# AkshayJha22/Cross-Sectional-Momentum-Strategy-Replication-Backtesting-Framework

Measured on AMD Instinct MI355X. Metric: asset-periods backtested/sec (1/2/4/8 GPU) + % HBM peak BW; decile match %, higher is better.
Workload: dtype f64

## Files before the change

### cross-sectional-momentum-strategy-replication-backtesting-framework_amd/csrc/signal.hip

```cpp
#include "csm_common.h"
#include "scan.h"
#include "shard.h"


#define PROBE_M 8
#define PROBE_DEN 8
__device__ __forceinline__ bool tail_probe(const double* __restrict__ P,
                                           const int64_t* __restrict__ month_start, int T_m,
                                           int64_t N, int64_t T_d) {
  static_assert(PROBE_M == 8, "the month spacing is a shift");
  const int lane = threadIdx.x & 63;
  const int64_t cs = N / 128;
  double x[PROBE_M][2];
  bool in[PROBE_M];
#pragma unroll
  for (int i = 0; i < PROBE_M; ++i) {
    const int m = (int)(((int64_t)(2 * i + 1) * T_m) >> 4);
    const int64_t d0 = month_start[m] < 0 ? 0 : month_start[m];
    const int64_t d1 = month_start[m + 1] < T_d ? month_start[m + 1] : T_d;
    in[i] = d1 > d0;
#pragma unroll
    for (int j = 0; j < 2; ++j)
      x[i][j] = in[i] ? P[(d1 - 1) * N + (2 * lane + j) * cs] : 0.0;
  }
  int gaps = 0, tot = 0;
#pragma unroll
  for (int i = 0; i < PROBE_M; ++i)
#pragma unroll
    for (int j = 0; j < 2; ++j) {
      gaps += __popcll(__ballot(in[i] && !(x[i][j] == x[i][j])));
      tot += in[i] ? 64 : 0;
    }
  return gaps * PROBE_DEN <= tot;
}

struct HaloArgs {
  int H, F, before, after;
  uint8_t* flags;
};
#define HALO_BATCH 8
template <int MAXD, int VEC, int NBUF, int BW, bool SH, bool BL, int JC = 0, bool HALO = false>
__global__ __launch_bounds__(64 * BW) void k_signal(
    const double* __restrict__ P, const int64_t* __restrict__ month_start, int T_m, int64_t N,
    int J, int skip, double* __restrict__ PMo, double* __restrict__ R, double* __restrict__ M,
    double* __restrict__ NR, const double* __restrict__ carry, const double* __restrict__ next_pm,
    double* __restrict__ carry_out, int64_t T_d, uint16_t* __restrict__ IDS, HaloArgs ha,
    int probe) {
  static_assert(!HALO || (SH && VEC == 2), "the halo prologue: shard passes, paired lanes");
  if (probe && tail_probe(P, month_start, T_m, N, T_d)) return;
  typedef typename RowT<VEC>::T VT;
  extern __shared__ __attribute__((aligned(16))) double ring_lds[];
  const int W = J + skip;
  const int tid = threadIdx.x;
  const int64_t a0 = ((int64_t)blockIdx.x * 64 * BW + tid) * VEC;
  const bool live = a0 < N;
  const int RS = 64 * VEC * BW;
  ScanLane sl[VEC];
  int* shc = reinterpret_cast<int*>(ring_lds + W * RS);
#pragma unroll
  for (int k = 0; k < VEC; ++k) {
    scan_init(sl[k], ring_lds + VEC * tid + k, RS, W, HALO ? nullptr : carry, N, a0 + k, live);
    if (SH) {
      shc[VEC * tid + k] = 0;
      shc[RS + VEC * tid + k] = -1;
      shc[2 * RS + VEC * tid + k] = -1;
    }
  }
  double npmh[VEC];
  if constexpr (HALO) {
    constexpr int HU = HALO_BATCH;
    const int64_t* ms = month_start;
    const int H = ha.H, F = ha.F, HF = H + F;
    const int64_t as = live ? a0 : 0;
    const int lane = tid & 63, wv = tid >> 6;
    const int64_t aw = a0 - 2 * lane;
    double* hpw = ring_lds + (size_t)W * RS + (size_t)(3 * RS) / 2;
    uint16_t* wl = reinterpret_cast<uint16_t*>(hpw + HU * RS) + wv * (HU * 128);
    int nh[VEC], fv[VEC], lv[VEC];
#pragma unroll
    for (int c = 0; c < VEC; ++c) { nh[c] = 0; fv[c] = -1; lv[c] = -1; npmh[c] = absent_val(); }
    for (int j0 = 0; j0 < HF; j0 += HU) {
      double2 xl[HU];
#pragma unroll
      for (int u = 0; u < HU; ++u) {
        const int j = j0 + u;
        const int m = j < H ? j : j + T_m;
        xl[u] = make_double2(absent_val(), absent_val());
        if (j < HF) {
          const int64_t d0 = ms[m], d1 = ms[m + 1];
          if (d1 > d0) xl[u] = *reinterpret_cast<const double2*>(P + (d1 - 1) * N + as);
        }
      }
      int nit = 0;
#pragma unroll
      for (int u = 0; u < HU; ++u) {
        *reinterpret_cast<double2*>(hpw + u * RS + 2 * tid) = xl[u];
#pragma unroll
        for (int c = 0; c < VEC; ++c) {
          const double x = comp(xl[u], c);
          const bool need = live && j0 + u < HF && !(x == x);
          const uint64_t mk = __ballot(need);
          if (need) wl[nit + lane_prefix(mk)] = (uint16_t)(u * 128 + 2 * lane + c);
          nit += __popcll(mk);
        }
      }
      __builtin_amdgcn_wave_barrier();
      for (int it0 = 0; it0 < nit; it0 += 128) {
        int item[2], u[2];
        int64_t d0[2], d1[2];
        double xs[2][HALO_WALK];
#pragma unroll
        for (int h = 0; h < 2; ++h) {
          const int it = it0 + 64 * h + lane;
          item[h] = it < nit ? (int)wl[it] : -1;
          u[h] = item[h] >> 7;
          const int j = j0 + (item[h] < 0 ? 0 : u[h]);
          const int m = j < H ? j : j + T_m;
          d0[h] = ms[m];
          d1[h] = ms[m + 1];
          const int64_t a = aw + (item[h] & 127);
#pragma unroll
          for (int k = 0; k < HALO_WALK; ++k) {
            const int64_t d = d1[h] - 2 - k;
            xs[h][k] = (item[h] >= 0 && d >= d0[h]) ? P[d * N + a] : absent_val();
          }
        }
#pragma unroll
        for (int h = 0; h < 2; ++h) {
          if (item[h] < 0) continue;
          const int64_t a = aw + (item[h] & 127);
          const double xlast = hpw[u[h] * RS + 128 * wv + (item[h] & 127)];
          bool p = !is_absent(xlast), got = false;
          double x = 0.0;
#pragma unroll
          for (int k = 0; k < HALO_WALK; ++k) {
            if (!got && xs[h][k] == xs[h][k]) { x = xs[h][k]; got = true; }
            p |= !is_absent(xs[h][k]);
          }
          if (!got && d1[h] - 1 - HALO_WALK > d0[h]) {
            const double y = halo_month_price(P, d0[h], d1[h] - 1 - HALO_WALK, N, a);
            if (y == y) { x = y; got = true; }
            p |= !is_absent(y);
          }
          hpw[u[h] * RS + 128 * wv + (item[h] & 127)] = got ? x : (p ? qnan() : absent_val());
        }
      }
      __syncthreads();
#pragma unroll
      for (int u = 0; u < HU; ++u) {
        const int j = j0 + u;
        if (j >= HF) break;
#pragma unroll
        for (int c = 0; c < VEC; ++c) {
          const double x = hpw[u * RS + 2 * tid + c];
          if (j < H) {
            if (live && !is_absent(x)) {
              if (!isnan_d(x)) { if (fv[c] < 0) fv[c] = nh[c]; lv[c] = nh[c]; }
              ++nh[c];
              scan_shadow(sl[c], x, j, ring_lds + VEC * tid + c, RS, W, J);
            }
          } else if (is_absent(npmh[c])) {
            npmh[c] = x;
          }
        }
      }
      __syncthreads();
    }
#pragma unroll
    for (int c = 0; c < VEC; ++c) {
      sl[c].prev = -1;
      uint8_t fl = 0;
      if (ha.before && !(fv[c] >= 0 && lv[c] - fv[c] >= W)) fl |= 1;
      if (ha.after && is_absent(npmh[c])) fl |= 2;
      if (live && ha.flags) ha.flags[a0 + c] = fl;
    }
    month_start += H;
  }
  const double* base = P + (live ? a0 : 0);
  const int64_t rstride = N;
  static_assert(!BL || VEC == 2, "buffer loads: paired lanes");
  const int voff = (int)((live ? a0 : 0) * 8);
  auto load_month = [&](VT (&buf)[MAXD], int mm) {
    mm = mm < T_m ? mm : T_m - 1;
    const int64_t f0 = month_start[mm], nn = month_start[mm + 1] - f0;
    if constexpr (BL) {
      typedef unsigned int u32x4 __attribute__((ext_vector_type(4)));
      const __amdgpu_buffer_rsrc_t rs = __builtin_amdgcn_make_buffer_rsrc(
          (void*)(P + f0 * N), (short)0, (int)(nn * N * 8), 0x00020000);
#pragma unroll
      for (int k = 0; k < MAXD; ++k) {
        const u32x4 w = __builtin_amdgcn_raw_buffer_load_b128(rs, voff + k * (int)(N * 8), 0, 0);
        buf[k] = *reinterpret_cast<const VT*>(&w);
      }
    } else {
      const int64_t pad = nn > 0 ? nn - 1 : (f0 > 0 ? -1 : 0);
#pragma unroll
      for (int k = 0; k < MAXD; ++k)
        buf[k] = *reinterpret_cast<const VT*>(base + (f0 + (k < nn ? k : pad)) * rstride);
    }
  };
  auto process = [&](const VT (&X)[MAXD], int m) {
    double pm[VEC];
    const int nnm = (int)(month_start[m + 1] - month_start[m]);
#pragma unroll
    for (int c = 0; c < VEC; ++c) {
      double last = 0.0;
      bool p = false, v = false;
#pragma unroll
      for (int k = 0; k < MAXD; ++k) {
        const double x = comp(X[k], c);
        const bool in = BL ? k < nnm : nnm > 0;
        const bool ok = in && x == x;
        p |= in && !is_absent(x);
        v |= ok;
        last = ok ? x : last;
      }
      pm[c] = p ? (v ? last : qnan()) : absent_val();
      if (SH && p) {
        int* q = shc + VEC * tid + c;
        q[0] += 1;
        if (q[RS] < 0) q[RS] = m;
        q[2 * RS] = m;
      }
    }
    if (live) {
      if (PMo && (!SH || shard_pm_kept(m, T_m, W))) {
        if (VEC == 2) *reinterpret_cast<double2*>(PMo + (int64_t)m * N + a0) = make_double2(pm[0], pm[VEC - 1]);
        else PMo[(int64_t)m * N + a0] = pm[0];
      }
      double mom[VEC];
      if constexpr (VEC == 2) {
        scan_step_pair<JC>(reinterpret_cast<ScanLane (&)[2]>(sl), reinterpret_cast<const double (&)[2]>(pm),
                       m, ring_lds + VEC * tid, RS, W, J, N, a0, R, M, NR,
                       reinterpret_cast<double (&)[2]>(mom));
      } else {
#pragma unroll
        for (int c = 0; c < VEC; ++c)
          mom[c] = scan_step(sl[c], pm[c], m, ring_lds + VEC * tid + c, RS, W, J, N, a0 + c, R, M, NR);
      }
      if (IDS) {
        if (VEC == 2)
          *reinterpret_cast<uint32_t*>(IDS + (int64_t)m * N + a0) =
              csm_fid(mom[0]) | (csm_fid(mom[VEC - 1]) << 16);
        else
          IDS[(int64_t)m * N + a0] = (uint16_t)csm_fid(mom[0]);
      }
    }
  };
  static_assert(NBUF == 2 || NBUF == 4, "two or four month buffers");
  VT A[MAXD], B[MAXD];
  if (NBUF == 2) {
    load_month(A, 0);
    for (int m = 0; m < T_m; m += 2) {
      load_month(B, m + 1);
      process(A, m);
      load_month(A, m + 2);
      if (m + 1 < T_m) process(B, m + 1);
    }
  } else {
    VT C[MAXD], D[MAXD];
    load_month(A, 0);
    load_month(B, 1);
    load_month(C, 2);
    for (int m = 0; m < T_m; m += 4) {
      load_month(D, m + 3);
      process(A, m);
      load_month(A, m + 4);
      if (m + 1 < T_m) process(B, m + 1);
      load_month(B, m + 5);
      if (m + 2 < T_m) process(C, m + 2);
      load_month(C, m + 6);
      if (m + 3 < T_m) process(D, m + 3);
    }
  }
  if (live) {
#pragma unroll
    for (int k = 0; k < VEC; ++k) {
      if constexpr (HALO) {
        if (sl[k].prev >= 0)
          NR[(int64_t)sl[k].prev * N + a0 + k] = pending_finish(npmh[k], sl[k].psff);
      } else {
        scan_finish(sl[k], ring_lds + VEC * tid + k, RS, W, N, a0 + k, NR, next_pm,
                    SH ? nullptr : carry_out);
      }
      if (SH) {
        const int* q = shc + VEC * tid + k;
        carry_out[a0 + k] = (double)q[0];
        carry_out[N + a0 + k] = (double)sl[k].prev;
        carry_out[2 * N + a0 + k] = sl[k].psff;
        carry_out[3 * N + a0 + k] = (double)q[RS];
        carry_out[4 * N + a0 + k] = (double)q[2 * RS];
      }
    }
  }
}

#define TAIL_U 8
#define TAIL_BACK 3

template <int MAXD, int BW, int JC>
__global__ __launch_bounds__(64 * BW) void k_signal_tail(
    const double* __restrict__ P, const int64_t* __restrict__ month_start, int T_m, int64_t N,
    int J, int skip, double* __restrict__ PMo, double* __restrict__ R, double* __restrict__ M,
    double* __restrict__ NR, const double* __restrict__ carry, const double* __restrict__ next_pm,
    double* __restrict__ carry_out, int64_t T_d, uint16_t* __restrict__ IDS,
    int probe) {
  if (probe && !tail_probe(P, month_start, T_m, N, T_d)) return;
  extern __shared__ __attribute__((aligned(16))) double ring_lds[];
  constexpr int U = TAIL_U, RS = 64 * BW, WA = 64;
  const int W = J + skip;
  const int tid = threadIdx.x, lane = tid & 63, wv = tid >> 6;
  const int64_t a0 = (int64_t)blockIdx.x * RS + tid;
  const bool live = a0 < N;
  const int64_t as = live ? a0 : 0;
  const int64_t aw = a0 - lane;
  const int64_t* ms = month_start;
  double* hp = ring_lds + (size_t)W * RS;
  double* hpw = hp + WA * wv;
  uint16_t* wl = reinterpret_cast<uint16_t*>(hp + U * RS) + wv * (2 * U * WA);
  uint16_t* wl2 = wl + U * WA;
  ScanLane sl;
  scan_init(sl, ring_lds + tid, RS, W, carry, N, a0, live);
  if (aw >= N) return;

  auto month_rows = [&](int m, int64_t& d0, int64_t& d1) {
    d0 = ms[m];
    d1 = ms[m + 1];
    d0 = d0 < 0 ? 0 : d0;
    d1 = d1 < T_d ? d1 : T_d;
  };
  auto load_last = [&](double (&xl)[U], int m0) {
#pragma unroll
    for (int u = 0; u < U; ++u) {
      xl[u] = absent_val();
      if (m0 + u < T_m) {
        int64_t d0, d1;
        month_rows(m0 + u, d0, d1);
        if (d1 > d0) xl[u] = P[(d1 - 1) * N + as];
      }
    }
  };
  auto fold = [&](double y, double& x, bool& got, bool& p) {
    if (!got && y == y) { x = y; got = true; }
    p |= !is_absent(y);
  };
  constexpr int K = MAXD - 1;
  struct Walk {
    int item, u, col;
    int64_t d0, d1;
    bool act;
  };
  auto issue = [&](auto& xs, Walk& w, const uint16_t* list, int it, int n, int m0) {
    constexpr int KK = sizeof(xs) / sizeof(double);
    w.act = it < n;
    w.item = w.act ? (int)list[it] : 0;
    w.u = w.item / WA;
    w.col = w.item % WA;
    month_rows(m0 + w.u, w.d0, w.d1);
    const int64_t a = aw + w.col;
#pragma unroll
    for (int k = 0; k < KK; ++k) {
      const int64_t d = w.d1 - 2 - k;
      xs[k] = (w.act && d >= w.d0) ? P[d * N + a] : absent_val();
    }
  };
  auto finish_back = [&](const double (&xs)[TAIL_BACK], const Walk& w, int& nb) {
    bool p = true, got = false;
    double x = 0.0;
#pragma unroll
    for (int k = 0; k < TAIL_BACK; ++k) fold(xs[k], x, got, p);
    const bool more = w.act && !got && w.d1 - 2 - TAIL_BACK >= w.d0;
    if (w.act && !more) hpw[w.u * RS + w.col] = got ? x : qnan();
    const uint64_t mk = __ballot(more);
    if (more) wl2[nb + lane_prefix(mk)] = (uint16_t)w.item;
    nb += __popcll(mk);
  };
  auto finish_month = [&](const double (&xs)[K], const Walk& w) {
    bool p = !is_absent(hpw[w.u * RS + w.col]), got = false;
    double x = 0.0;
#pragma unroll
    for (int k = 0; k < K; ++k) fold(xs[k], x, got, p);
    if (w.act) hpw[w.u * RS + w.col] = got ? x : (p ? qnan() : absent_val());
  };
  auto walk_months = [&](int i0, int n, int m0) {
    double XS[K], XT[K];
    Walk wb, wc;
    const bool two = i0 + 64 < n;
    issue(XS, wb, wl2, i0 + lane, n, m0);
    if (two) issue(XT, wc, wl2, i0 + 64 + lane, n, m0);
    finish_month(XS, wb);
    if (two) finish_month(XT, wc);
  };

  double xa[U], xb[U];
  load_last(xa, 0);
  for (int m0 = 0; m0 < T_m; m0 += U) {
    load_last(xb, m0 + U);
    int na = 0, nb = 0;
#pragma unroll
    for (int u = 0; u < U; ++u) {
      hp[u * RS + tid] = xa[u];
      bool in = false;
      if (m0 + u < T_m) {
        int64_t d0, d1;
        month_rows(m0 + u, d0, d1);
        in = d1 > d0;
      }
      const double x = xa[u];
      const bool need = live && in && !(x == x);
      const bool nb_ = need && is_absent(x), na_ = need && !nb_;
      const uint64_t mka = __ballot(na_), mkb = __ballot(nb_);
      const int item = u * WA + lane;
      if (na_) wl[na + lane_prefix(mka)] = (uint16_t)item;
      if (nb_) wl2[nb + lane_prefix(mkb)] = (uint16_t)item;
      na += __popcll(mka);
      nb += __popcll(mkb);
    }
    __builtin_amdgcn_wave_barrier();
    if (na + nb > 0) {
      double xs[TAIL_BACK];
      Walk wa;
      int db = nb < 128 ? nb : 128;
      issue(xs, wa, wl, lane, na, m0);
      walk_months(0, db, m0);
      finish_back(xs, wa, nb);
      for (int it0 = 64; it0 < na; it0 += 64) {
        issue(xs, wa, wl, it0 + lane, na, m0);
        finish_back(xs, wa, nb);
      }
      __builtin_amdgcn_wave_barrier();
      for (; db < nb; db += 128) walk_months(db, nb, m0);
    }
    __builtin_amdgcn_wave_barrier();
#pragma unroll 1
    for (int u = 0; u < U; ++u) {
      const int m = m0 + u;
      if (m >= T_m) break;
      if (!live) continue;
      const double pm = hp[u * RS + tid];
      if (PMo) PMo[(int64_t)m * N + a0] = pm;
      const double mom = scan_step<JC>(sl, pm, m, ring_lds + tid, RS, W, J, N, a0, R, M, NR);
      if (IDS) IDS[(int64_t)m * N + a0] = (uint16_t)csm_fid(mom);
    }
    __builtin_amdgcn_wave_barrier();
#pragma unroll
    for (int u = 0; u < U; ++u) xa[u] = xb[u];
  }
  if (live) scan_finish(sl, ring_lds + tid, RS, W, N, a0, NR, next_pm, carry_out);
}

static int g_tune_signal_vec = 2;
static int g_tune_signal_bwf = 0;
static int g_tune_signal_tail = 2;
static int g_tune_signal_j12 = 1;
#define SIGNAL_BWF_MIN_N (180 * 512)
static const TuneKnob g_knobs[] = {
    {"signal_vec", &g_tune_signal_vec, [](int v) { return v == 1 || v == 2; }},
    {"signal_bwf", &g_tune_signal_bwf, [](int v) { return v == 0 || v == 1 || v == 4; }},
    {"signal_j12", &g_tune_signal_j12, [](int v) { return v == 0 || v == 1; }},
    {"signal_tail", &g_tune_signal_tail, [](int v) { return v >= 0 && v <= 2; }},
};
int csm_tune_signal(const char* key, int value) { return tune_set(g_knobs, key, value); }

int signal_launch(csm_ctx* ctx, const char* who, const double* P, int64_t T_d, int64_t N,
                  const int64_t* month_start, int32_t T_m, int32_t max_month_days, int32_t J,
                  int32_t skip, double* PM, double* R, double* M, double* NR, const double* carry,
                  const double* next_pm, double* carry_out, bool sh, uint16_t* ids,
                  const HaloArgs* halo) {
  int r = prep(ctx);
  if (r) return r;
  if (sh && (!PM || !carry_out || T_m < 1))
    return set_err(ctx, CSM_E_INVAL, "%s: a shard pass needs PM and state, and at least one month",
                   who);
  if (!P || !month_start || !M || !NR || N <= 0 || T_d < 0 || T_m < 0 || J < 1 || skip < 0 ||
      J + skip > 256 || max_month_days < 1)
    return set_err(ctx, CSM_E_INVAL, "%s: bad arguments (N=%lld T_m=%d J=%d skip=%d)", who,
                   (long long)N, T_m, J, skip);
  if (max_month_days > 32)
    return set_err(ctx, CSM_E_INVAL, "%s: months longer than 32 days are not supported "
                   "(use csm_month_end + csm_momentum)", who);
  if (T_m == 0) return CSM_OK;
  if (T_d == 0)
    return set_err(ctx, CSM_E_INVAL, "%s: %d months and no day row", who, T_m);
  const int W = J + skip;
  const bool can2 = (N % 2 == 0) && aligned16(P) && (!PM || aligned16(PM)) && aligned16(M) &&
                    aligned16(NR) && (!R || aligned16(R));
  const int vec = (g_tune_signal_vec == 1 || !can2) ? 1 : 2;
  const size_t tlds = (size_t)(W + TAIL_U) * 128 * sizeof(double) + (size_t)2 * TAIL_U * 128 * sizeof(uint16_t);
  int tail = (!sh && !halo && can2 && tlds <= 160 * 1024) ? g_tune_signal_tail : 0;
  if (tail == 2 && N < (int64_t)SIGNAL_BWF_MIN_N) tail = 1;
  int probe_ = tail == 2;
  if (tail != 0) {
    const bool d23 = max_month_days <= 23, j12 = J == 12;
    const void* fn =
        d23 ? (j12 ? (const void*)k_signal_tail<23, 2, 12> : (const void*)k_signal_tail<23, 2, 0>)
            : (j12 ? (const void*)k_signal_tail<32, 2, 12> : (const void*)k_signal_tail<32, 2, 0>);
    if (tlds > 65536)
      HIP_CHECK(ctx, hipFuncSetAttribute(fn, hipFuncAttributeMaxDynamicSharedMemorySize, (int)tlds));
    const unsigned blocks = (unsigned)((N + 127) / 128);
    int T_m_ = T_m, J_ = J, skip_ = skip;
    int64_t N_ = N, T_d_ = T_d;
    void* args[] = {(void*)&P, (void*)&month_start, &T_m_, &N_, &J_, &skip_, (void*)&PM, (void*)&R,
                    (void*)&M, (void*)&NR, (void*)&carry, (void*)&next_pm, (void*)&carry_out, &T_d_,
                    (void*)&ids, &probe_};
    HIP_CHECK(ctx, hipLaunchKernel(fn, dim3(blocks), dim3(128), args, tlds, ctx->stream));
    LAUNCH_CHECK(ctx, who);
    if (tail == 1) return CSM_OK;
  }
  const bool fits4 = vec == 2 && max_month_days <= 23 && N * 8 * 32 < ((int64_t)1 << 31);
  const bool wide4 = fits4 && (g_tune_signal_bwf == 4 ||
                               (g_tune_signal_bwf == 0 && N >= (int64_t)SIGNAL_BWF_MIN_N));
  const int bw = wide4 ? 4 : 1;
  const size_t lds = (size_t)W * 64 * vec * bw * sizeof(double) +
                     (sh ? (size_t)3 * 64 * vec * bw * sizeof(int) : 0) +
                     (halo ? (size_t)HALO_BATCH * 64 * vec * bw * sizeof(double) +
                             (size_t)bw * HALO_BATCH * 128 * sizeof(uint16_t) : 0);
  const unsigned blocks = (unsigned)((N / vec + 64 * bw - 1) / (64 * bw));
  const void* fn = nullptr;
#define SIG1(V, SH_)                                                                            \
  (max_month_days <= 23 && V == 2 ? (const void*)k_signal<23, V, 4, 1, SH_, false>              \
   : max_month_days <= 24         ? (const void*)k_signal<24, V, 4, 1, SH_, false>              \
                                  : (const void*)k_signal<32, V, 4, 1, SH_, false>)
  const bool j12 = sh && J == 12 && g_tune_signal_j12;
  if (halo && !(sh && wide4))
    return set_err(ctx, CSM_E_INVAL, "%s: the fused halo prologue runs in the wide shard kernel "
                   "(even N >= %d, months of <= 23 days); use csm_shard_halo + "
                   "csm_signal_shard_halo", who, SIGNAL_BWF_MIN_N);
  if (halo)
    fn = j12 ? (const void*)k_signal<23, 2, 2, 4, true, true, 12, true>
             : (const void*)k_signal<23, 2, 2, 4, true, true, 0, true>;
  else if (wide4 && j12)
    fn = (const void*)k_signal<23, 2, 2, 4, true, true, 12>;
  else if (wide4)
    fn = sh ? (const void*)k_signal<23, 2, 2, 4, true, true> : (const void*)k_signal<23, 2, 2, 4, false, true>;
  else if (vec == 2)
    fn = sh ? SIG1(2, true) : SIG1(2, false);
  else
    fn = sh ? SIG1(1, true) : SIG1(1, false);
#undef SIG1
  if (lds > 65536)
    HIP_CHECK(ctx, hipFuncSetAttribute(fn, hipFuncAttributeMaxDynamicSharedMemorySize, (int)lds));
  {
    int T_m_ = T_m, J_ = J, skip_ = skip;
    int64_t N_ = N, T_d_ = T_d;
    HaloArgs ha = halo ? *halo : HaloArgs{0, 0, 0, 0, nullptr};
    void* args[] = {(void*)&P, (void*)&month_start, &T_m_, &N_, &J_, &skip_, (void*)&PM, (void*)&R,
                    (void*)&M, (void*)&NR, (void*)&carry, (void*)&next_pm, (void*)&carry_out, &T_d_,
                    (void*)&ids, (void*)&ha, &probe_};
    HIP_CHECK(ctx, hipLaunchKernel(fn, dim3(blocks), dim3(64 * bw), args, lds, ctx->stream));
  }
  LAUNCH_CHECK(ctx, who);
  return CSM_OK;
}

extern "C" {

int csm_signal(csm_ctx* ctx, const double* P, int64_t T_d, int64_t N, const int64_t* month_start,
               int32_t T_m, int32_t max_month_days, int32_t J, int32_t skip, double* PM, double* R,
               double* M, double* NR, const double* carry, const double* next_pm,
               double* carry_out) {
  return signal_launch(ctx, "csm_signal", P, T_d, N, month_start, T_m, max_month_days, J,
                       skip, PM, R, M, NR, carry, next_pm, carry_out);
}

int csm_signal_ids(csm_ctx* ctx, const double* P, int64_t T_d, int64_t N,
                   const int64_t* month_start, int32_t T_m, int32_t max_month_days,
                   int32_t min_month_days, int32_t J, int32_t skip, double* PM, double* R,
                   double* M, double* NR, uint16_t* ids) {
  if (!ids || (N % 4) != 0 || ((uintptr_t)ids & 7u) != 0)
    return set_err(ctx, CSM_E_INVAL, "csm_signal_ids: ids must be non-NULL and 8-B aligned, N %% 4 == 0 "
                   "(N=%lld)", (long long)N);
  (void)min_month_days;
  return signal_launch(ctx, "csm_signal_ids", P, T_d, N, month_start, T_m, max_month_days, J,
                       skip, PM, R, M, NR, nullptr, nullptr, nullptr, false, ids);
}

int csm_signal_shard(csm_ctx* ctx, const double* P, int64_t T_d, int64_t N,
                     const int64_t* month_start, int32_t T_m, int32_t max_month_days, int32_t J,
                     int32_t skip, double* PM, double* R, double* M, double* NR, double* state) {
  return signal_launch(ctx, "csm_signal_shard", P, T_d, N, month_start, T_m,
                       max_month_days, J, skip, PM, R, M, NR, nullptr, nullptr, state, true);
}

int csm_signal_shard_ids(csm_ctx* ctx, const double* P, int64_t T_d, int64_t N,
                         const int64_t* month_start, int32_t T_m, int32_t max_month_days,
                         int32_t J, int32_t skip, double* PM, double* R, double* M, double* NR,
                         double* state, uint16_t* ids) {
  if (!ids || (N % 4) != 0 || ((uintptr_t)ids & 7u) != 0)
    return set_err(ctx, CSM_E_INVAL, "csm_signal_shard_ids: needs ids, N %% 4 == 0, 8-B aligned ids");
  return signal_launch(ctx, "csm_signal_shard_ids", P, T_d, N, month_start, T_m,
                       max_month_days, J, skip, PM, R, M, NR, nullptr, nullptr, state, true, ids);
}

int csm_signal_halo(csm_ctx* ctx, const double* P, int64_t T_d, int64_t N,
                    const int64_t* month_start, int32_t H, int32_t T_m, int32_t F, int32_t before,
                    int32_t after, int32_t max_month_days, int32_t J, int32_t skip, double* PM,
                    double* R, double* M, double* NR, double* state, uint16_t* ids,
                    uint8_t* flags) {
  if (!flags || H < 0 || F < 0 || F > 8 || J + skip > 64)
    return set_err(ctx, CSM_E_INVAL, "csm_signal_halo: bad arguments (flags [N], H >= 0, "
                   "0 <= F <= 8, J + skip <= 64)");
  if (ids && ((N % 4) != 0 || ((uintptr_t)ids & 7u) != 0))
    return set_err(ctx, CSM_E_INVAL, "csm_signal_halo: ids need N %% 4 == 0, 8-B alignment");
  const HaloArgs ha{H, F, before ? 1 : 0, after ? 1 : 0, flags};
  return signal_launch(ctx, "csm_signal_halo", P, T_d, N, month_start, T_m, max_month_days, J,
                       skip, PM, R, M, NR, nullptr, nullptr, state, true, ids, &ha);
}

int csm_signal_shard_halo(csm_ctx* ctx, const double* P, int64_t T_d, int64_t N,
                          const int64_t* month_start, int32_t T_m, int32_t max_month_days,
                          int32_t J, int32_t skip, const double* carry, const double* next_pm,
                          double* PM, double* R, double* M, double* NR, double* state,
                          uint16_t* ids) {
  if (!carry || !next_pm)
    return set_err(ctx, CSM_E_INVAL, "csm_signal_shard_halo: needs the halo's carry and next_pm");
  if (ids && ((N % 4) != 0 || ((uintptr_t)ids & 7u) != 0))
    return set_err(ctx, CSM_E_INVAL, "csm_signal_shard_halo: ids need N %% 4 == 0, 8-B alignment");
  return signal_launch(ctx, "csm_signal_shard_halo", P, T_d, N, month_start, T_m, max_month_days,
                       J, skip, PM, R, M, NR, carry, next_pm, state, true, ids);
}

}
```

Measured before the change: 823.2 billion.

## Split signal tail kernel into producer loader waves and consumer scanner waves

The tail kernel now uses separate wave roles. Loader waves gather each month's last-valid prices into a double-buffered LDS staging area. Scanner waves then run the momentum scan on the previous batch, with block-level barriers handing each batch from loaders to scanners, so the gather latency overlaps the scan work. Day indices are narrowed to 32-bit, and a waves-per-EU occupancy hint is added. This costs twice the staging LDS, more threads per block and a __syncthreads per batch, and adds a guard that T_d fits in 32 bits.

```diff
diff --git a/cross-sectional-momentum-strategy-replication-backtesting-framework_amd/csrc/signal.hip b/cross-sectional-momentum-strategy-replication-backtesting-framework_amd/csrc/signal.hip
--- a/cross-sectional-momentum-strategy-replication-backtesting-framework_amd/csrc/signal.hip
+++ b/cross-sectional-momentum-strategy-replication-backtesting-framework_amd/csrc/signal.hip
@@ -297,46 +297,87 @@
 
 #define TAIL_U 8
 #define TAIL_BACK 3
-
-template <int MAXD, int BW, int JC>
-__global__ __launch_bounds__(64 * BW) void k_signal_tail(
+constexpr int TAIL_NS = 2;
+constexpr int TAIL_NL = 2;
+constexpr int TAIL_CPL = 1;
+constexpr int tail_waves_per_simd(int nw) { return nw == 4 ? 4 : 3; }
+
+template <int MAXD, int NS, int NL, int CPL, int JC>
+__global__ __launch_bounds__(64 * (NS + NL))
+__attribute__((amdgpu_waves_per_eu(tail_waves_per_simd(NS + NL)))) void k_signal_tail(
     const double* __restrict__ P, const int64_t* __restrict__ month_start, int T_m, int64_t N,
     int J, int skip, double* __restrict__ PMo, double* __restrict__ R, double* __restrict__ M,
     double* __restrict__ NR, const double* __restrict__ carry, const double* __restrict__ next_pm,
     double* __restrict__ carry_out, int64_t T_d, uint16_t* __restrict__ IDS,
     int probe) {
+  static_assert(NS % NL == 0 && (CPL == 1 || CPL == 2), "whole 64-column groups per loader wave");
   if (probe && !tail_probe(P, month_start, T_m, N, T_d)) return;
   extern __shared__ __attribute__((aligned(16))) double ring_lds[];
-  constexpr int U = TAIL_U, RS = 64 * BW, WA = 64;
+  constexpr int U = TAIL_U, RS = 64 * NS, CW = RS / NL, CP = CW / 64;
+  static_assert(U * CW <= 65536, "list items are 16-bit");
   const int W = J + skip;
-  const int tid = threadIdx.x, lane = tid & 63, wv = tid >> 6;
-  const int64_t a0 = (int64_t)blockIdx.x * RS + tid;
-  const bool live = a0 < N;
-  const int64_t as = live ? a0 : 0;
-  const int64_t aw = a0 - lane;
+  const int tid = threadIdx.x, lane = tid & 63;
+  const int wv = __builtin_amdgcn_readfirstlane(tid >> 6);
+  const bool scanner = wv < NS;
+  const int nbat = (T_m + U - 1) / U;
   const int64_t* ms = month_start;
   double* hp = ring_lds + (size_t)W * RS;
-  double* hpw = hp + WA * wv;
-  uint16_t* wl = reinterpret_cast<uint16_t*>(hp + U * RS) + wv * (2 * U * WA);
-  uint16_t* wl2 = wl + U * WA;
-  ScanLane sl;
-  scan_init(sl, ring_lds + tid, RS, W, carry, N, a0, live);
-  if (aw >= N) return;
-
-  auto month_rows = [&](int m, int64_t& d0, int64_t& d1) {
-    d0 = ms[m];
-    d1 = ms[m + 1];
-    d0 = d0 < 0 ? 0 : d0;
-    d1 = d1 < T_d ? d1 : T_d;
-  };
-  auto load_last = [&](double (&xl)[U], int m0) {
+  if (scanner) {
+    const int64_t a0 = (int64_t)blockIdx.x * RS + tid;
+    const bool live = a0 < N;
+    ScanLane sl;
+    scan_init(sl, ring_lds + tid, RS, W, carry, N, a0, live);
+    for (int k = 0; k <= nbat; ++k) {
+      if (k > 0 && live) {
+        const int m0 = (k - 1) * U;
+        const double* hb = hp + ((k - 1) & 1) * (U * RS) + tid;
+#pragma unroll 1
+        for (int u = 0; u < U; ++u) {
+          const int m = m0 + u;
+          if (m >= T_m) break;
+          const double pm = hb[u * RS];
+          if (PMo) PMo[(int64_t)m * N + a0] = pm;
+          const double mom = scan_step<JC>(sl, pm, m, ring_lds + tid, RS, W, J, N, a0, R, M, NR);
+          if (IDS) IDS[(int64_t)m * N + a0] = (uint16_t)csm_fid(mom);
+        }
+      }
+      if (k < nbat) __syncthreads();
+    }
+    if (live) scan_finish(sl, ring_lds + tid, RS, W, N, a0, NR, next_pm, carry_out);
+    return;
+  }
+  const int lw = wv - NS;
+  const int64_t aw = (int64_t)blockIdx.x * RS + (int64_t)lw * CW;
+  const bool wlive = aw < N;
+  bool lv[CP];
+  int64_t as[CP];
+#pragma unroll
+  for (int c = 0; c < CP; ++c) {
+    const int64_t a = aw + 64 * c + lane;
+    lv[c] = wlive && a < N;
+    as[c] = lv[c] ? a : 0;
+  }
+  double* hpw = hp + CW * lw;
+  uint16_t* wl = reinterpret_cast<uint16_t*>(hp + 2 * U * RS) + lw * (2 * U * CW);
+  uint16_t* wl2 = wl + U * CW;
+
+  auto month_rows = [&](int m, int& d0, int& d1) {
+    const int64_t e0 = ms[m], e1 = ms[m + 1];
+    d0 = (int)(e0 < 0 ? 0 : (e0 < T_d ? e0 : T_d));
+    d1 = (int)(e1 < T_d ? (e1 < 0 ? 0 : e1) : T_d);
+  };
+  auto load_last = [&](double (&xl)[U][CP], int m0) {
 #pragma unroll
     for (int u = 0; u < U; ++u) {
-      xl[u] = absent_val();
+#pragma unroll
+      for (int c = 0; c < CP; ++c) xl[u][c] = absent_val();
       if (m0 + u < T_m) {
-        int64_t d0, d1;
+        int d0, d1;
         month_rows(m0 + u, d0, d1);
-        if (d1 > d0) xl[u] = P[(d1 - 1) * N + as];
+        if (d1 > d0) {
+#pragma unroll
+          for (int c = 0; c < CP; ++c) xl[u][c] = P[(int64_t)(d1 - 1) * N + as[c]];
+        }
       }
     }
   };
@@ -347,21 +388,21 @@
   constexpr int K = MAXD - 1;
   struct Walk {
     int item, u, col;
-    int64_t d0, d1;
+    int d0, d1;
     bool act;
   };
   auto issue = [&](auto& xs, Walk& w, const uint16_t* list, int it, int n, int m0) {
     constexpr int KK = sizeof(xs) / sizeof(double);
     w.act = it < n;
     w.item = w.act ? (int)list[it] : 0;
-    w.u = w.item / WA;
-    w.col = w.item % WA;
+    w.u = w.item / CW;
+    w.col = w.item % CW;
     month_rows(m0 + w.u, w.d0, w.d1);
     const int64_t a = aw + w.col;
 #pragma unroll
     for (int k = 0; k < KK; ++k) {
-      const int64_t d = w.d1 - 2 - k;
-      xs[k] = (w.act && d >= w.d0) ? P[d * N + a] : absent_val();
+      const int d = w.d1 - 2 - k;
+      xs[k] = (w.act && d >= w.d0) ? P[(int64_t)d * N + a] : absent_val();
     }
   };
   auto finish_back = [&](const double (&xs)[TAIL_BACK], const Walk& w, int& nb) {
@@ -383,70 +424,70 @@
     if (w.act) hpw[w.u * RS + w.col] = got ? x : (p ? qnan() : absent_val());
   };
   auto walk_months = [&](int i0, int n, int m0) {
-    double XS[K], XT[K];
-    Walk wb, wc;
-    const bool two = i0 + 64 < n;
+    double XS[K];
+    Walk wb;
     issue(XS, wb, wl2, i0 + lane, n, m0);
-    if (two) issue(XT, wc, wl2, i0 + 64 + lane, n, m0);
-    finish_month(XS, wb);
-    if (two) finish_month(XT, wc);
-  };
-
-  double xa[U], xb[U];
-  load_last(xa, 0);
-  for (int m0 = 0; m0 < T_m; m0 += U) {
-    load_last(xb, m0 + U);
-    int na = 0, nb = 0;
-#pragma unroll
-    for (int u = 0; u < U; ++u) {
-      hp[u * RS + tid] = xa[u];
-      bool in = false;
-      if (m0 + u < T_m) {
-        int64_t d0, d1;
-        month_rows(m0 + u, d0, d1);
-        in = d1 > d0;
-      }
-      const double x = xa[u];
-      const bool need = live && in && !(x == x);
-      const bool nb_ = need && is_absent(x), na_ = need && !nb_;
-      const uint64_t mka = __ballot(na_), mkb = __ballot(nb_);
-      const int item = u * WA + lane;
-      if (na_) wl[na + lane_prefix(mka)] = (uint16_t)item;
-      if (nb_) wl2[nb + lane_prefix(mkb)] = (uint16_t)item;
-      na += __popcll(mka);
-      nb += __popcll(mkb);
-    }
-    __builtin_amdgcn_wave_barrier();
-    if (na + nb > 0) {
-      double xs[TAIL_BACK];
-      Walk wa;
-      int db = nb < 128 ? nb : 128;
-      issue(xs, wa, wl, lane, na, m0);
-      walk_months(0, db, m0);
-      finish_back(xs, wa, nb);
-      for (int it0 = 64; it0 < na; it0 += 64) {
-        issue(xs, wa, wl, it0 + lane, na, m0);
+    if constexpr (CPL == 2) {
+      double XT[K];
+      Walk wc;
+      const bool two = i0 + 64 < n;
+      if (two) issue(XT, wc, wl2, i0 + 64 + lane, n, m0);
+      finish_month(XS, wb);
+      if (two) finish_month(XT, wc);
+    } else {
+      finish_month(XS, wb);
+    }
+  };
+
+  double xa[U][CP];
+  if (wlive) load_last(xa, 0);
+  for (int k = 0; k < nbat; ++k) {
+    if (wlive) {
+      const int m0 = k * U;
+      hpw = hp + (k & 1) * (U * RS) + CW * lw;
+      int na = 0, nb = 0;
+#pragma unroll
+      for (int u = 0; u < U; ++u) {
+        bool in = false;
+        if (m0 + u < T_m) {
+          int d0, d1;
+          month_rows(m0 + u, d0, d1);
+          in = d1 > d0;
+        }
+#pragma unroll
+        for (int c = 0; c < CP; ++c) {
+          const double x = xa[u][c];
+          hpw[u * RS + 64 * c + lane] = x;
+          const bool need = lv[c] && in && !(x == x);
+          const bool nb_ = need && is_absent(x), na_ = need && !nb_;
+          const uint64_t mka = __ballot(na_), mkb = __ballot(nb_);
+          const int item = u * CW + 64 * c + lane;
+          if (na_) wl[na + lane_prefix(mka)] = (uint16_t)item;
+          if (nb_) wl2[nb + lane_prefix(mkb)] = (uint16_t)item;
+          na += __popcll(mka);
+          nb += __popcll(mkb);
+        }
+      }
+      load_last(xa, m0 + U);
+      __builtin_amdgcn_wave_barrier();
+      if (na + nb > 0) {
+        double xs[TAIL_BACK];
+        Walk wa;
+        constexpr int TRIP = 64 * CPL;
+        int db = nb < TRIP ? nb : TRIP;
+        issue(xs, wa, wl, lane, na, m0);
+        walk_months(0, db, m0);
         finish_back(xs, wa, nb);
-      }
-      __builtin_amdgcn_wave_barrier();
-      for (; db < nb; db += 128) walk_months(db, nb, m0);
-    }
-    __builtin_amdgcn_wave_barrier();
-#pragma unroll 1
-    for (int u = 0; u < U; ++u) {
-      const int m = m0 + u;
-      if (m >= T_m) break;
-      if (!live) continue;
-      const double pm = hp[u * RS + tid];
-      if (PMo) PMo[(int64_t)m * N + a0] = pm;
-      const double mom = scan_step<JC>(sl, pm, m, ring_lds + tid, RS, W, J, N, a0, R, M, NR);
-      if (IDS) IDS[(int64_t)m * N + a0] = (uint16_t)csm_fid(mom);
-    }
-    __builtin_amdgcn_wave_barrier();
-#pragma unroll
-    for (int u = 0; u < U; ++u) xa[u] = xb[u];
-  }
-  if (live) scan_finish(sl, ring_lds + tid, RS, W, N, a0, NR, next_pm, carry_out);
+        for (int it0 = 64; it0 < na; it0 += 64) {
+          issue(xs, wa, wl, it0 + lane, na, m0);
+          finish_back(xs, wa, nb);
+        }
+        __builtin_amdgcn_wave_barrier();
+        for (; db < nb; db += TRIP) walk_months(db, nb, m0);
+      }
+    }
+    __syncthreads();
+  }
 }
 
 static int g_tune_signal_vec = 2;
@@ -486,24 +527,28 @@
   const bool can2 = (N % 2 == 0) && aligned16(P) && (!PM || aligned16(PM)) && aligned16(M) &&
                     aligned16(NR) && (!R || aligned16(R));
   const int vec = (g_tune_signal_vec == 1 || !can2) ? 1 : 2;
-  const size_t tlds = (size_t)(W + TAIL_U) * 128 * sizeof(double) + (size_t)2 * TAIL_U * 128 * sizeof(uint16_t);
-  int tail = (!sh && !halo && can2 && tlds <= 160 * 1024) ? g_tune_signal_tail : 0;
+  constexpr int TRS = 64 * TAIL_NS;
+  const size_t tlds = (size_t)(W + 2 * TAIL_U) * TRS * sizeof(double) +
+                      (size_t)2 * TAIL_U * TRS * sizeof(uint16_t);
+  int tail = (!sh && !halo && can2 && tlds <= 160 * 1024 && T_d < ((int64_t)1 << 31))
+                 ? g_tune_signal_tail : 0;
   if (tail == 2 && N < (int64_t)SIGNAL_BWF_MIN_N) tail = 1;
   int probe_ = tail == 2;
   if (tail != 0) {
     const bool d23 = max_month_days <= 23, j12 = J == 12;
-    const void* fn =
-        d23 ? (j12 ? (const void*)k_signal_tail<23, 2, 12> : (const void*)k_signal_tail<23, 2, 0>)
-            : (j12 ? (const void*)k_signal_tail<32, 2, 12> : (const void*)k_signal_tail<32, 2, 0>);
+#define TAILK(D, JC_) (const void*)k_signal_tail<D, TAIL_NS, TAIL_NL, TAIL_CPL, JC_>
+    const void* fn = d23 ? (j12 ? TAILK(23, 12) : TAILK(23, 0)) : (j12 ? TAILK(32, 12) : TAILK(32, 0));
+#undef TAILK
     if (tlds > 65536)
       HIP_CHECK(ctx, hipFuncSetAttribute(fn, hipFuncAttributeMaxDynamicSharedMemorySize, (int)tlds));
-    const unsigned blocks = (unsigned)((N + 127) / 128);
+    const unsigned blocks = (unsigned)((N + TRS - 1) / TRS);
     int T_m_ = T_m, J_ = J, skip_ = skip;
     int64_t N_ = N, T_d_ = T_d;
     void* args[] = {(void*)&P, (void*)&month_start, &T_m_, &N_, &J_, &skip_, (void*)&PM, (void*)&R,
                     (void*)&M, (void*)&NR, (void*)&carry, (void*)&next_pm, (void*)&carry_out, &T_d_,
                     (void*)&ids, &probe_};
-    HIP_CHECK(ctx, hipLaunchKernel(fn, dim3(blocks), dim3(128), args, tlds, ctx->stream));
+    HIP_CHECK(ctx, hipLaunchKernel(fn, dim3(blocks), dim3(64 * (TAIL_NS + TAIL_NL)), args, tlds,
+                                   ctx->stream));
     LAUNCH_CHECK(ctx, who);
     if (tail == 1) return CSM_OK;
   }
```

After: 866.7 billion (median of 6 runs). 1.05x the previous value.
